# wangty537/raft_optical_flow

Hardware: AMD Instinct MI355X
Metric: image-pairs/s at Sintel 436x1024, 32 iters; corr-lookup GB/s vs HBM peak (higher is better)
Workload: dtype fp32 (convs: f16x3 split MFMA, fp32 accumulate); 1 GPU; RAFT-full inference, 436x1024 padded to 440x1024, 1 pair(s)/GPU/step, iters=32, all-pairs corr, hipGraph; global_batch=1, parallelism=frame-pair sharding x1

## Files before the change

### raft_optical_flow_amd/csrc/lookup_conv.hip

```cpp
#include "lookup_common.hpp"

namespace raft {
namespace {

constexpr int LC_TH = 2, LC_TW = 16, LC_M = 32;
constexpr int LC_R = 4, LC_L = 4, LC_RD = 9;
constexpr int LC_NTAP = LC_L * LC_RD * LC_RD;
constexpr int LC_KS = (LC_NTAP + 31) / 32;
constexpr int LC_N = 256;
constexpr int LC_F1N = 128;
constexpr int LC_F1K = 7, LC_F1KK = 49;
constexpr int LC_F1KS = (2 * LC_F1KK + 31) / 32;
constexpr int LC_FPH = LC_TH + LC_F1K - 1, LC_FPW = LC_TW + LC_F1K - 1;
constexpr int LC_PX = 4;

constexpr int LC_A_BYTES = LC_KS * LC_M * 128;
constexpr int LC_A1_BYTES = LC_F1KS * LC_M * 128;
constexpr int LC_FL_BYTES = LC_FPH * LC_FPW * 8;
constexpr int LC_PATCH_FLOATS = 16 * patch_rs<4>();
constexpr int LC_PATCH_BYTES = 8 * 2 * LC_PATCH_FLOATS * 4;
constexpr int LC_YT_BYTES = 8 * LC_PX * LC_L * LC_RD * 16;
constexpr int LC_OFF_A1 = LC_A_BYTES, LC_OFF_FL = LC_OFF_A1 + LC_A1_BYTES, LC_OFF_PATCH = LC_OFF_FL + LC_FL_BYTES,
              LC_OFF_YT = LC_OFF_PATCH + LC_PATCH_BYTES, LC_LDS = LC_OFF_YT + LC_YT_BYTES;
static_assert(LC_LDS <= 160 * 1024, "LDS budget");

struct LookupConvArgs {
  LookupArgs a;
  const h8* wfrag;
  const float* bias;
  float* out;
  int out_ld;
  int* out_flag;
  const h8* f1frag;
  const float* f1bias;
  float* f1out;
  int f1out_ld;
  int* f1flag;
  int tx_n, ty_n;
  int span_slot;
};

constexpr int LC_SPAN_SLOTS = 256;
__device__ unsigned long long g_lc_span[2 * LC_SPAN_SLOTS];
int g_lc_span_next = -1;

__device__ __forceinline__ void wave_sync() {
  __builtin_amdgcn_fence(__ATOMIC_RELEASE, "wavefront");
  __builtin_amdgcn_wave_barrier();
  __builtin_amdgcn_fence(__ATOMIC_ACQUIRE, "wavefront");
}

template <bool X3, bool BF>
__device__ __forceinline__ void split1(float x, _Float16& hi, _Float16& lo) {
  if constexpr (BF) {
    hi = __builtin_bit_cast(_Float16, (__bf16)x);
  } else {
    hi = (_Float16)x;
    if constexpr (X3) lo = (_Float16)(x - (float)hi);
  }
}

#ifdef LC_STAMPS
__device__ unsigned long long g_lcstamp[16 * 16384];
__device__ __forceinline__ unsigned long long lc_clock() {
  unsigned long long t;
  __builtin_amdgcn_sched_barrier(0);
  asm volatile("s_memtime %0\n\ts_waitcnt lgkmcnt(0)" : "=s"(t)::"memory");
  __builtin_amdgcn_sched_barrier(0);
  return t;
}
__device__ __forceinline__ unsigned long long lc_real() {
  unsigned long long t;
  __builtin_amdgcn_sched_barrier(0);
  asm volatile("s_memrealtime %0\n\ts_waitcnt lgkmcnt(0)" : "=s"(t)::"memory");
  __builtin_amdgcn_sched_barrier(0);
  return t;
}
#define LC_STAMP(k) lc_t[k] = lc_clock()
#else
#define LC_STAMP(k)
#endif

template <int PREC>
__global__ __launch_bounds__(512) void lookup_conv_kernel(LookupConvArgs g) {
#ifdef LC_STAMPS
  unsigned long long lc_t[10];
  const unsigned long long lc_r0 = lc_real();
  LC_STAMP(0);
#endif
  constexpr bool X3 = PREC == RAFT_PREC_F16X3;
  constexpr bool BF = PREC == RAFT_PREC_BF16;
  constexpr int NT = X3 ? 4 : 2;
  constexpr int R = LC_R, RD = LC_RD, WD = 2 * R + 2, RS = patch_rs<4>();
  __shared__ __attribute__((aligned(1024))) char smem[LC_LDS];
  const LookupArgs& a = g.a;
  const int lane = threadIdx.x & 63;
  const int wv = __builtin_amdgcn_readfirstlane(threadIdx.x >> 6);
  const int tile = xcd_tile(blockIdx.x, gridDim.x);
  if (g.span_slot >= 0 && threadIdx.x == 0)
    atomicMin(&g_lc_span[2 * g.span_slot], (unsigned long long)__builtin_amdgcn_s_memrealtime());
  const int per = g.tx_n * g.ty_n;
  const int b = tile / per, sr = tile - b * per;
  const int y0 = (sr / g.tx_n) * LC_TH, x0 = (sr % g.tx_n) * LC_TW;
  const int H = a.H, W = a.W, P = H * W;

  constexpr int LC_PF = 3;
  constexpr int PF = LC_PF;
  h8 wb[PF + 1][NT];
  auto load_w = [&](int j, h8 (&dst)[NT]) {
    const h8* wf = j < LC_KS ? g.wfrag + ((j * (LC_N / 32) + wv) * 4) * 64
                             : g.f1frag + (((j - LC_KS) * (LC_F1N / 32) + wv) * 4) * 64;
#pragma unroll
    for (int t = 0; t < NT; ++t) dst[t] = wf[t * 64 + lane];
  };

  const int ti = lane >> 4, tj = (lane >> 2) & 3, rr = lane & 3;
  const int lrow = ti * 4 + rr;
  int lth[LC_L], ltw[LC_L];
  unsigned lmsz[LC_L];
  const float* lbs[LC_L];
#pragma unroll
  for (int l = 0; l < LC_L; ++l) {
    lth[l] = a.lv[l].th;
    ltw[l] = a.lv[l].tw;
    lmsz[l] = (unsigned)a.lv[l].mapsz;
    lbs[l] = a.lbase[l];
  }
  float px_x[LC_PX], px_y[LC_PX];
  int px_gp[LC_PX];
  bool px_ok[LC_PX];
#pragma unroll
  for (int k = 0; k < LC_PX; ++k) {
    const int mk = LC_PX * wv + k;
    const int yy = y0 + (mk >> 4), xx = x0 + (mk & 15);
    const bool ok = yy < H && xx < W;
    px_ok[k] = ok;
    px_gp[k] = ok ? b * P + yy * W + xx : b * P;
  }
  {
    int gk = px_gp[0];
#pragma unroll
    for (int k = 1; k < LC_PX; ++k) gk = (lane & 3) == k ? px_gp[k] : gk;
    const float cx = a.coords[2L * gk], cy = a.coords[2L * gk + 1];
#pragma unroll
    for (int k = 0; k < LC_PX; ++k) {
      px_x[k] = __int_as_float(__builtin_amdgcn_readlane(__float_as_int(cx), k));
      px_y[k] = __int_as_float(__builtin_amdgcn_readlane(__float_as_int(cy), k));
    }
  }
#ifdef LC_STAMPS
  asm volatile("" ::"v"(px_x[0]), "v"(px_y[LC_PX - 1]));
  LC_STAMP(7);
#endif
  const bool col = lane < LC_L * RD;
  int lq = 0;
#pragma unroll
  for (int k = 1; k < LC_L; ++k) lq += lane >= k * RD ? 1 : 0;
  const int l = col ? lq : 0;
  const int ix = lane - l * RD;
  const f32x4 prm = a.prm[l];
  const int fi = threadIdx.x;
  const int fyy = y0 - 3 + fi / LC_FPW, fxx = x0 - 3 + fi % LC_FPW;
  const bool fin = fi < LC_FPH * LC_FPW && (unsigned)fyy < (unsigned)H && (unsigned)fxx < (unsigned)W;
  f32x2 fc = {0.f, 0.f};
  if (fin) fc = *reinterpret_cast<const f32x2*>(a.coords + 2L * ((long)b * P + fyy * W + fxx));
  const int m = lane & 31, h = lane >> 5;
  const float c1b = g.bias ? g.bias[32 * wv + m] : 0.f;
  const float f1b = (wv < 4 && g.f1bias) ? g.f1bias[32 * wv + m] : 0.f;
  asm volatile("" ::"v"(prm), "v"(c1b), "v"(f1b), "v"(fc));

  __builtin_amdgcn_sched_barrier(0);
  f32x4 v[LC_PX][LC_L];
  bool off32 = true;
  const unsigned nmaps = (unsigned)(a.B * P);
#pragma unroll
  for (int l = 0; l < LC_L; ++l) off32 &= (unsigned long long)nmaps * lmsz[l] * 4ull < 0x7FFFFFF0ull;
  if (off32) {
    __amdgpu_buffer_rsrc_t rsl[LC_L];
    unsigned lano[LC_L], lmsz4[LC_L];
#pragma unroll
    for (int l = 0; l < LC_L; ++l) {
      rsl[l] = __builtin_amdgcn_make_buffer_rsrc(const_cast<float*>(lbs[l]), (short)0, (int)(nmaps * lmsz[l] * 4u),
                                                 0x00020000);
      lano[l] = __umul24((unsigned)ti, (unsigned)(64 * ltw[l])) + 16u * (unsigned)(lane & 15);
      lmsz4[l] = lmsz[l] * 4u;
    }
    int t_sb, t_row, t_col;
    {
      const int ik = (lane >> 2) & 3, il = lane & 3;
      float fx = px_x[0], fy = px_y[0];
      int gpk = px_gp[0];
      bool okk = px_ok[0];
#pragma unroll
      for (int k = 1; k < LC_PX; ++k) {
        fx = ik == k ? px_x[k] : fx;
        fy = ik == k ? px_y[k] : fy;
        gpk = ik == k ? px_gp[k] : gpk;
        okk = ik == k ? px_ok[k] : okk;
      }
      int thl = lth[0], twl = ltw[0];
      unsigned msl = lmsz4[0];
#pragma unroll
      for (int l = 1; l < LC_L; ++l) {
        thl = il == l ? lth[l] : thl;
        twl = il == l ? ltw[l] : twl;
        msl = il == l ? lmsz4[l] : msl;
      }
      const int wx0 = (floor_origin(fx) >> il) - R, wy0 = (floor_origin(fy) >> il) - R;
      const int tyo = wy0 >> 2, txo = wx0 >> 2;
      const int ntx = ((wx0 + WD - 1) >> 2) - txo + 1;
      const int rlo = max(wy0, 0), rhi = min(wy0 + WD, 4 * thl);
      const int clo = max(txo, 0), chi = min(txo + ntx, twl);
      const int rn = okk ? max(rhi - rlo, 0) : 0, cn = max(chi - clo, 0);
      t_sb = (int)((unsigned)gpk * msl + (unsigned)(tyo * twl + txo) * 64u);
      t_row = ((rlo - 4 * tyo) & 0xFFFF) | (rn << 16);
      t_col = ((clo - txo) & 0xFFFF) | (cn << 16);
    }
#pragma unroll
    for (int k = 0; k < LC_PX; ++k) {
#pragma unroll
      for (int l = 0; l < LC_L; ++l) {
        const unsigned sb = (unsigned)__builtin_amdgcn_readlane(t_sb, 4 * k + l);
        const int rp = __builtin_amdgcn_readlane(t_row, 4 * k + l), cp = __builtin_amdgcn_readlane(t_col, 4 * k + l);
        const bool tok = ((unsigned)(lrow - (rp & 0xFFFF)) < (unsigned)(rp >> 16)) &
                         ((unsigned)(tj - (cp & 0xFFFF)) < (unsigned)(cp >> 16));
        unsigned offv = sb + lano[l];
        asm volatile("" : "+v"(offv));
        const unsigned off = tok ? offv : 0x80000000u;
        v[k][l] = __builtin_bit_cast(f32x4, __builtin_amdgcn_raw_buffer_load_b128(rsl[l], off, 0, 0));
      }
    }
  } else {
    int t_lo, t_hi, t_row, t_col;
    {
      const int ik = (lane >> 2) & 3, il = lane & 3;
      float fx = px_x[0], fy = px_y[0];
      int gpk = px_gp[0];
      bool okk = px_ok[0];
#pragma unroll
      for (int k = 1; k < LC_PX; ++k) {
        fx = ik == k ? px_x[k] : fx;
        fy = ik == k ? px_y[k] : fy;
        gpk = ik == k ? px_gp[k] : gpk;
        okk = ik == k ? px_ok[k] : okk;
      }
      int thl = lth[0], twl = ltw[0];
      unsigned msl = lmsz[0];
      const float* bsl = lbs[0];
#pragma unroll
      for (int l = 1; l < LC_L; ++l) {
        thl = il == l ? lth[l] : thl;
        twl = il == l ? ltw[l] : twl;
        msl = il == l ? lmsz[l] : msl;
        bsl = il == l ? lbs[l] : bsl;
      }
      const int wx0 = (floor_origin(fx) >> il) - R, wy0 = (floor_origin(fy) >> il) - R;
      const int tyo = wy0 >> 2, txo = wx0 >> 2;
      const int ntx = ((wx0 + WD - 1) >> 2) - txo + 1;
      const int rlo = max(wy0, 0), rhi = min(wy0 + WD, 4 * thl);
      const int clo = max(txo, 0), chi = min(txo + ntx, twl);
      const int rn = okk ? max(rhi - rlo, 0) : 0, cn = max(chi - clo, 0);
      const float* wbase = bsl + (long)((unsigned long long)(unsigned)gpk * msl) + ((long)tyo * twl + txo) * 16;
      const unsigned long long wa = reinterpret_cast<unsigned long long>(wbase);
      t_lo = (int)(unsigned)wa;
      t_hi = (int)(unsigned)(wa >> 32);
      t_row = ((rlo - 4 * tyo) & 0xFFFF) | (rn << 16);
      t_col = ((clo - txo) & 0xFFFF) | (cn << 16);
    }
#pragma unroll
    for (int k = 0; k < LC_PX; ++k) {
#pragma unroll
      for (int l = 0; l < LC_L; ++l) {
        const unsigned lo = (unsigned)__builtin_amdgcn_readlane(t_lo, 4 * k + l);
        const unsigned hi = (unsigned)__builtin_amdgcn_readlane(t_hi, 4 * k + l);
        const int rp = __builtin_amdgcn_readlane(t_row, 4 * k + l), cp = __builtin_amdgcn_readlane(t_col, 4 * k + l);
        const bool tok = ((unsigned)(lrow - (rp & 0xFFFF)) < (unsigned)(rp >> 16)) &
                         ((unsigned)(tj - (cp & 0xFFFF)) < (unsigned)(cp >> 16));
        const float* wbase = reinterpret_cast<const float*>(((unsigned long long)hi << 32) | lo);
        const __amdgpu_buffer_rsrc_t rs =
            __builtin_amdgcn_make_buffer_rsrc(const_cast<float*>(wbase), (short)0, 0x7FFFFFFF, 0x00020000);
        unsigned offv = __umul24((unsigned)ti, (unsigned)(64 * ltw[l])) + 16u * (unsigned)(lane & 15);
        asm volatile("" : "+v"(offv));
        const unsigned off = tok ? offv : 0x80000000u;
        v[k][l] = __builtin_bit_cast(f32x4, __builtin_amdgcn_raw_buffer_load_b128(rs, off, 0, 0));
      }
    }
  }
  LC_STAMP(1);
  int4* ytab = reinterpret_cast<int4*>(smem + LC_OFF_YT) + wv * LC_PX * LC_L * RD;
  int xw[LC_PX], xi[LC_PX];
  float xt[LC_PX];
  bool onp[LC_PX];
#pragma unroll
  for (int k = 0; k < LC_PX; ++k) {
    const float s = __builtin_ldexpf(1.0f, -l);
    const int xf = __builtin_amdgcn_readfirstlane(floor_origin(px_x[k]));
    const int yf = __builtin_amdgcn_readfirstlane(floor_origin(px_y[k]));
    axis_entry<R>(px_x[k] * s, xf >> l, ix, prm[0], prm[1], xw[k], xt[k], xi[k]);
    int yw, yi;
    float yt;
    axis_entry<R, true>(px_y[k] * s, yf >> l, ix, prm[2], prm[3], yw, yt, yi);
    onp[k] = xw[k] >= 0 && yw >= 0;
    if (col) ytab[k * LC_L * RD + lane] = int4{yw >= 0 ? yw * RS * 4 : yw, __float_as_int(yt), __float_as_int(1.0f - yt), yi};
  }
  float2* fl = reinterpret_cast<float2*>(smem + LC_OFF_FL);
  if (fi < LC_FPH * LC_FPW) {
    float2 fv = {0.f, 0.f};
    if (fin) {
      fv.x = fc[0] - (float)fxx;
      fv.y = fc[1] - (float)fyy;
    }
    fl[fi] = fv;
  }
  LC_STAMP(2);

#pragma unroll
  for (int j = 0; j < PF; ++j) load_w(j, wb[j]);
  char* Abase = smem;
  bool big = false;
  auto patch_of = [&](int k) {
    return reinterpret_cast<float*>(smem + LC_OFF_PATCH) + (wv * 2 + (k & 1)) * LC_PATCH_FLOATS;
  };
  const int cbase = l * RD * RD + ix * RD;
  auto taps = [&](int k, float (&val)[RD]) {
    const float* patch = patch_of(k);
    const int4* yt = ytab + k * LC_L * RD;
    const float ex = 1.0f - xt[k];
    const int xwk = xw[k];
    if (__all(!col || onp[k])) {
      if (col) {
        const char* p0 = reinterpret_cast<const char*>(&patch[pidx<4>(0, xwk, l)]);
        const char* p1 = reinterpret_cast<const char*>(&patch[pidx<4>(0, xwk + 1, l)]);
        auto at = [](const char* bp, int byte) { return *reinterpret_cast<const float*>(bp + byte); };
        int ro[RD];
        float tyv[RD];
        bool cons = true;
#pragma unroll
        for (int iy = 0; iy < RD; ++iy) {
          const int2 ye = *reinterpret_cast<const int2*>(&yt[l * RD + iy]);
          ro[iy] = ye.x;
          tyv[iy] = __int_as_float(ye.y);
        }
#pragma unroll
        for (int iy = 1; iy < RD; ++iy) cons &= ro[iy] == ro[0] + iy * (4 * RS);
        if (__all(cons)) {
          const char* q0 = p0 + ro[0];
          const char* q1 = p1 + ro[0];
          float a0[RD + 1], a1[RD + 1];
#pragma unroll
          for (int r = 0; r <= RD; ++r) {
            a0[r] = at(q0, r * (4 * RS));
            a1[r] = at(q1, r * (4 * RS));
          }
#pragma unroll
          for (int iy = 0; iy < RD; ++iy) {
            const float ty = tyv[iy], sS = 1.0f - ty;
            const f32x2 c0 = {a0[iy], a0[iy + 1]}, c1 = {a1[iy], a1[iy + 1]};
            const f32x2 hh = __builtin_elementwise_fma(c0, (f32x2){ex, ex}, c1 * (f32x2){xt[k], xt[k]});
            val[iy] = fmaf(sS, hh.x, ty * hh.y);
          }
        } else {
#pragma unroll
          for (int iy = 0; iy < RD; ++iy) {
            const float ty = tyv[iy], sS = 1.0f - ty;
            const f32x2 c0 = {at(p0, ro[iy]), at(p0, ro[iy] + 4 * RS)}, c1 = {at(p1, ro[iy]), at(p1, ro[iy] + 4 * RS)};
            const f32x2 hh = __builtin_elementwise_fma(c0, (f32x2){ex, ex}, c1 * (f32x2){xt[k], xt[k]});
            val[iy] = fmaf(sS, hh.x, ty * hh.y);
          }
        }
      }
    } else if (col) {
      unsigned deferred = 0;
#pragma unroll
      for (int iy = 0; iy < RD; ++iy) {
        const int4 ye = yt[l * RD + iy];
        const int yw2 = ye.x;
        const float ty = __int_as_float(ye.y), sS = __int_as_float(ye.z);
        const bool on = (xwk | yw2) >= 0;
        const bool nan = xwk == NAN_POS || yw2 == NAN_POS;
        const int r0 = on ? yw2 / (4 * RS) : 0, c0 = on ? xwk : 0;
        const float vv = patch[pidx<4>(r0, c0, l)] * (sS * ex) + patch[pidx<4>(r0, c0 + 1, l)] * (sS * xt[k]) +
                         patch[pidx<4>(r0 + 1, c0, l)] * (ty * ex) + patch[pidx<4>(r0 + 1, c0 + 1, l)] * (ty * xt[k]);
        val[iy] = nan ? __builtin_nanf("") : vv;
        deferred |= (!on && !nan) ? 1u << iy : 0u;
      }
      if (deferred != 0) {
        const Level& lvl = a.lv[l];
        const float* mp = a.pyr + lvl.off + (long)px_gp[k] * lvl.mapsz;
        auto at = [&](int yy, int xx) {
          return ((unsigned)yy < (unsigned)lvl.h && (unsigned)xx < (unsigned)lvl.w) ? mp[tiled_index(yy, xx, lvl.tw)]
                                                                                    : 0.f;
        };
#pragma unroll
        for (int iy = 0; iy < RD; ++iy) {
          if (!((deferred >> iy) & 1u)) continue;
          const int4 ye = yt[l * RD + iy];
          const int yi = ye.w;
          const float ty = __int_as_float(ye.y), sS = __int_as_float(ye.z);
          val[iy] = at(yi, xi[k]) * (sS * ex) + at(yi, xi[k] + 1) * (sS * xt[k]) + at(yi + 1, xi[k]) * (ty * ex) +
                    at(yi + 1, xi[k] + 1) * (ty * xt[k]);
        }
      }
    }
  };
  auto write_row = [&](int k, const float (&val)[RD]) {
    const int mk = LC_PX * wv + k;
    const int sw = (mk >> 1) & 7;
    if (col) {
      const int par = cbase & 1;
      float vv[RD];
#pragma unroll
      for (int iy = 0; iy < RD; ++iy) {
        vv[iy] = px_ok[k] ? val[iy] : 0.f;
        big |= fabsf(vv[iy]) > RAFT_RANGE_LIMIT;
      }
      auto at_c = [&](int c, int half) {
        const int j = c >> 5, kk = c & 31;
        return Abase + j * (LC_M * 128) + mk * 128 + (((4 * half + (kk >> 3)) ^ sw) << 4) + 2 * (kk & 7);
      };
#pragma unroll
      for (int q = 0; q < 4; ++q) {
        const float a0 = par ? vv[2 * q + 1] : vv[2 * q], a1 = par ? vv[2 * q + 2] : vv[2 * q + 1];
        _Float16 h0, l0, h1, l1;
        split1<X3, BF>(a0, h0, l0);
        split1<X3, BF>(a1, h1, l1);
        const int c = cbase + 2 * q + par;
        *reinterpret_cast<h2*>(at_c(c, 0)) = h2{h0, h1};
        if constexpr (X3) *reinterpret_cast<h2*>(at_c(c, 1)) = h2{l0, l1};
      }
      {
        const float a = par ? vv[0] : vv[RD - 1];
        _Float16 hs, ls;
        split1<X3, BF>(a, hs, ls);
        const int c = cbase + (par ? 0 : RD - 1);
        *reinterpret_cast<_Float16*>(at_c(c, 0)) = hs;
        if constexpr (X3) *reinterpret_cast<_Float16*>(at_c(c, 1)) = ls;
      }
    } else if (lane - LC_L * RD < 32 * LC_KS - LC_NTAP) {
      const int c = LC_NTAP + lane - LC_L * RD;
      const int j = c >> 5, kk = c & 31;
      char* rb = Abase + j * (LC_M * 128) + mk * 128;
      *reinterpret_cast<_Float16*>(rb + (((kk >> 3) ^ sw) << 4) + 2 * (kk & 7)) = (_Float16)0.f;
      if constexpr (X3) *reinterpret_cast<_Float16*>(rb + (((4 + (kk >> 3)) ^ sw) << 4) + 2 * (kk & 7)) = (_Float16)0.f;
    }
    if (a.flow && lane < 2 && px_ok[k]) {
      const int p = px_gp[k] - b * P;
      const float gcoord = lane == 0 ? (float)(p % W) : (float)(p / W);
      a.flow[(long)px_gp[k] * a.flow_ld + lane] = (lane == 0 ? px_x[k] : px_y[k]) - gcoord;
    }
  };
#pragma unroll
  for (int k = 0; k < LC_PX; k += 2) {
#pragma unroll
    for (int lv_ = 0; lv_ < LC_L; ++lv_) {
      *reinterpret_cast<f32x4*>(&patch_of(k)[pidx<4>(lrow, tj * 4, lv_)]) = v[k][lv_];
      *reinterpret_cast<f32x4*>(&patch_of(k + 1)[pidx<4>(lrow, tj * 4, lv_)]) = v[k + 1][lv_];
    }
    wave_sync();
    float va[RD], vb[RD];
    taps(k, va);
    taps(k + 1, vb);
    write_row(k, va);
    write_row(k + 1, vb);
    wave_sync();
  }
  if (a.range_flag && big) *a.range_flag = 1;
  LC_STAMP(3);
  __syncthreads();
  {
    const int mm = threadIdx.x >> 4, q = threadIdx.x & 15;
    const int py = mm >> 4, px = mm & 15;
    float e[8];
#pragma unroll
    for (int i = 0; i < 8; ++i) {
      const int k = 8 * q + i, t = k >> 1;
      const int dy = t / LC_F1K, dx = t - dy * LC_F1K;
      const float2 fv = fl[(py + (k < 2 * LC_F1KK ? dy : 0)) * LC_FPW + px + (k < 2 * LC_F1KK ? dx : 0)];
      e[i] = k < 2 * LC_F1KK ? ((k & 1) ? fv.y : fv.x) : 0.f;
    }
    h8 hi, lo;
    split8<X3, BF>(f32x4{e[0], e[1], e[2], e[3]}, f32x4{e[4], e[5], e[6], e[7]}, hi, lo);
    const int j = q >> 2, qd = q & 3, sw = (mm >> 1) & 7;
    char* row = smem + LC_OFF_A1 + j * (LC_M * 128) + mm * 128;
    *reinterpret_cast<h8*>(row + ((qd ^ sw) << 4)) = hi;
    if constexpr (X3) *reinterpret_cast<h8*>(row + (((4 + qd) ^ sw) << 4)) = lo;
  }
  __syncthreads();
  LC_STAMP(4);

  const int sw = (m >> 1) & 7;
  f32x16 acc = {}, accx = {}, facc = {}, faccx = {};
  const bool f1w = wv < LC_F1N / 32;
  struct AF {
    h8 ah[2], al[2];
  };
  auto read_af = [&](const char* A, AF& f) {
    const char* row = A + m * 128;
#pragma unroll
    for (int qq = 0; qq < 2; ++qq) {
      f.ah[qq] = *reinterpret_cast<const h8*>(row + (((2 * h + qq) ^ sw) << 4));
      if constexpr (X3) f.al[qq] = *reinterpret_cast<const h8*>(row + (((4 + 2 * h + qq) ^ sw) << 4));
    }
  };
  auto mfma_af = [&](const AF& f, const h8 (&B)[NT], f32x16& c, f32x16& cx) {
#pragma unroll
    for (int qq = 0; qq < 2; ++qq) {
      if constexpr (BF) {
        c = __builtin_amdgcn_mfma_f32_32x32x16_bf16(__builtin_bit_cast(bf8, f.ah[qq]), __builtin_bit_cast(bf8, B[qq]),
                                                    c, 0, 0, 0);
      } else {
        c = __builtin_amdgcn_mfma_f32_32x32x16_f16(f.ah[qq], B[qq], c, 0, 0, 0);
      }
      if constexpr (X3) {
        cx = __builtin_amdgcn_mfma_f32_32x32x16_f16(f.ah[qq], B[2 + qq], cx, 0, 0, 0);
        c = __builtin_amdgcn_mfma_f32_32x32x16_f16(f.al[qq], B[qq], c, 0, 0, 0);
      }
    }
  };
  auto load_w_any = [&](int j, h8 (&dst)[NT]) {
    const int wq = j < LC_KS ? wv : (wv < LC_F1N / 32 ? wv : LC_F1N / 32 - 1);
    const h8* wf = j < LC_KS ? g.wfrag + ((j * (LC_N / 32) + wq) * 4) * 64
                             : g.f1frag + (((j - LC_KS) * (LC_F1N / 32) + wq) * 4) * 64;
#pragma unroll
    for (int t = 0; t < NT; ++t) dst[t] = wf[t * 64 + lane];
  };
  constexpr int NRA = X3 ? 4 : 2, NMA = X3 ? 6 : 2;
  auto groups = [&](bool loads) {
    if (loads) __builtin_amdgcn_sched_group_barrier(0x020, NT, 0);
#pragma unroll
    for (int i = 0; i < NMA; ++i) {
      if (i < NRA) __builtin_amdgcn_sched_group_barrier(0x100, 1, 0);
      __builtin_amdgcn_sched_group_barrier(0x008, 1, 0);
    }
  };
  AF af[2];
  read_af(Abase, af[0]);
#pragma unroll
  for (int j = 0; j < LC_KS; ++j) {
    __builtin_amdgcn_sched_barrier(0);
    if (j + PF < LC_KS + LC_F1KS) load_w_any(j + PF, wb[(j + PF) % (PF + 1)]);
    read_af(j + 1 < LC_KS ? Abase + (j + 1) * (LC_M * 128) : smem + LC_OFF_A1, af[(j + 1) & 1]);
    mfma_af(af[j & 1], wb[j % (PF + 1)], acc, accx);
    groups(j + PF < LC_KS + LC_F1KS);
    __builtin_amdgcn_sched_barrier(0);
  }
  if (f1w) {
#pragma unroll
    for (int j = LC_KS; j < LC_KS + LC_F1KS; ++j) {
      __builtin_amdgcn_sched_barrier(0);
      if (j + PF < LC_KS + LC_F1KS) load_w_any(j + PF, wb[(j + PF) % (PF + 1)]);
      if (j + 1 < LC_KS + LC_F1KS) read_af(smem + LC_OFF_A1 + (j + 1 - LC_KS) * (LC_M * 128), af[(j + 1) & 1]);
      mfma_af(af[j & 1], wb[j % (PF + 1)], facc, faccx);
      __builtin_amdgcn_sched_barrier(0);
    }
  }
  if constexpr (X3) {
#pragma unroll
    for (int r = 0; r < 16; ++r) {
      acc[r] += accx[r] * (1.0f / SPLIT_SCALE);
      facc[r] += faccx[r] * (1.0f / SPLIT_SCALE);
    }
  }
#ifdef LC_STAMPS
  asm volatile("" ::"v"(acc[0]), "v"(acc[15]), "v"(facc[0]));
#endif
  LC_STAMP(5);

  auto store = [&](const f32x16& c, float bias, float* out, int ld, int n, int* flag) {
    bool obig = false;
#pragma unroll
    for (int r = 0; r < 16; ++r) {
      const int mm = (r & 3) + 8 * (r >> 2) + 4 * h;
      const int yy = y0 + (mm >> 4), xx = x0 + (mm & 15);
      const float o = fmaxf(c[r] + bias, 0.f);
      if (yy < H && xx < W) {
        obig |= o > RAFT_RANGE_LIMIT;
        out[((long)b * P + yy * W + xx) * ld + n] = o;
      }
    }
    if (flag && obig) *flag = 1;
  };
  store(acc, c1b, g.out, g.out_ld, 32 * wv + m, g.out_flag);
  if (wv < LC_F1N / 32) store(facc, f1b, g.f1out, g.f1out_ld, 32 * wv + m, g.f1flag);
  if (g.span_slot >= 0) {
    __builtin_amdgcn_s_waitcnt(0);
    __syncthreads();
    if (threadIdx.x == 0)
      atomicMax(&g_lc_span[2 * g.span_slot + 1], (unsigned long long)__builtin_amdgcn_s_memrealtime());
  }
#ifdef LC_STAMPS
  __builtin_amdgcn_s_waitcnt(0);
  LC_STAMP(6);
  const unsigned long long lc_r1 = lc_real();
  const unsigned wid = blockIdx.x * 8 + wv;
  if (lane == 0 && wid < 16384) {
    unsigned long long* gs = g_lcstamp + wid * 16;
    gs[0] = lc_r0;
    gs[1] = lc_r1;
    for (int k = 0; k < 7; ++k) gs[2 + k] = lc_t[k];
    gs[9] = lc_t[7];
  }
#endif
}

__global__ void lookup_conv_pack_kernel(const h8* __restrict__ split, int k_steps, int nsub, h8* __restrict__ out) {
  const int i = blockIdx.x * blockDim.x + threadIdx.x;
  const int total = k_steps * nsub * 4 * 64;
  if (i >= total) return;
  const int lane = i & 63, t = (i >> 6) & 3, rest = i >> 8;
  const int s = rest % nsub, j = rest / nsub;
  const int n = 32 * s + (lane & 31), hh = lane >> 5, qq = t & 1, lo = t >> 1;
  out[i] = split[((long)n * k_steps + j) * 8 + lo * 4 + 2 * hh + qq];
}

}
}

using namespace raft;

#ifdef LC_STAMPS
extern "C" int raft_debug_lcstamps(unsigned long long* host, int n) {
  return (int)hipMemcpyFromSymbol(host, HIP_SYMBOL(g_lcstamp), sizeof(unsigned long long) * (size_t)n);
}
#endif

extern "C" size_t raft_lookup_conv_weight_floats(int n, int k_pad) {
  if (n <= 0 || n % 32 || k_pad <= 0) return 0;
  return (size_t)((k_pad + 31) / 32) * (size_t)n * 32;
}

extern "C" int raft_lookup_conv_pack_weight(const void* split_weight, int n_pad, int k_pad, int n, void* out,
                                            raft_stream_t stream) {
  RAFT_REQUIRE(split_weight && out && n > 0 && n % 32 == 0 && n <= n_pad && k_pad > 0 && k_pad % 32 == 0,
               "raft_lookup_conv_pack_weight: bad arguments");
  RAFT_REQUIRE((((uintptr_t)split_weight | (uintptr_t)out) & 15) == 0, "raft_lookup_conv_pack_weight: 16-B alignment");
  const int ks = k_pad / 32, nsub = n / 32;
  const int total = ks * nsub * 256;
  hipLaunchKernelGGL(lookup_conv_pack_kernel, dim3((unsigned)cdiv(total, 256)), dim3(256), 0, as_stream(stream),
                     reinterpret_cast<const h8*>(split_weight), ks, nsub, reinterpret_cast<h8*>(out));
  return check_launch("raft_lookup_conv_pack_weight");
}

extern "C" int raft_corr_lookup_conv(const float* pyramid, int B, int H, int W, int L, int radius, const float* coords,
                                     float* flow_out, int flow_ld, int* range_flag, int precision,
                                     const void* c1_weight, const float* c1_bias, int c1_n, float* c1_out,
                                     int c1_out_ld, int* c1_range_flag, const void* f1_weight, const float* f1_bias,
                                     int f1_n, int f1_k, float* f1_out, int f1_out_ld, int* f1_range_flag,
                                     raft_stream_t stream) {
  RAFT_REQUIRE(L == LC_L && radius == LC_R, "raft_corr_lookup_conv: radius 4 and 4 levels only (got %d, %d)", radius,
               L);
  RAFT_REQUIRE(c1_n == LC_N && f1_n == LC_F1N && f1_k == LC_F1K,
               "raft_corr_lookup_conv: convc1 256 / convf1 128 outputs, convf1 7x7 only");
  RAFT_REQUIRE(precision == RAFT_PREC_F16X3 || precision == RAFT_PREC_F16 || precision == RAFT_PREC_BF16,
               "raft_corr_lookup_conv: precision must be F16X3, F16 or BF16 (got %d)", precision);
  RAFT_REQUIRE(c1_weight && c1_out && c1_out_ld >= c1_n && f1_weight && f1_out && f1_out_ld >= f1_n,
               "raft_corr_lookup_conv: bad conv arguments");
  RAFT_REQUIRE((((uintptr_t)c1_weight | (uintptr_t)f1_weight) & 15) == 0 && ((uintptr_t)coords & 7) == 0,
               "raft_corr_lookup_conv: 16-B aligned weights, 8-B aligned coords");
  LookupConvArgs g;
  int rc = lookup_args(g.a, pyramid, B, H, W, L, radius, coords, 0, c1_out, LC_NTAP, 0, flow_out, flow_ld, range_flag);
  if (rc) return rc;
  g.wfrag = reinterpret_cast<const h8*>(c1_weight);
  g.bias = c1_bias;
  g.out = c1_out;
  g.out_ld = c1_out_ld;
  g.out_flag = c1_range_flag;
  g.f1frag = reinterpret_cast<const h8*>(f1_weight);
  g.f1bias = f1_bias;
  g.f1out = f1_out;
  g.f1out_ld = f1_out_ld;
  g.f1flag = f1_range_flag;
  g.tx_n = cdiv(W, LC_TW);
  g.ty_n = cdiv(H, LC_TH);
  hipStreamCaptureStatus cap = hipStreamCaptureStatusNone;
  const bool capturing = hipStreamIsCapturing(as_stream(stream), &cap) == hipSuccess && cap != hipStreamCaptureStatusNone;
  g.span_slot = !capturing && g_lc_span_next >= 0 && g_lc_span_next < LC_SPAN_SLOTS ? g_lc_span_next++ : -1;
  const long nt = (long)B * g.tx_n * g.ty_n;
  RAFT_REQUIRE(nt < (1L << 31), "raft_corr_lookup_conv: grid too large");
  hipStream_t s = as_stream(stream);
  const dim3 grid((unsigned)nt);
  if (precision == RAFT_PREC_F16X3)
    hipLaunchKernelGGL(lookup_conv_kernel<RAFT_PREC_F16X3>, grid, dim3(512), 0, s, g);
  else if (precision == RAFT_PREC_F16)
    hipLaunchKernelGGL(lookup_conv_kernel<RAFT_PREC_F16>, grid, dim3(512), 0, s, g);
  else
    hipLaunchKernelGGL(lookup_conv_kernel<RAFT_PREC_BF16>, grid, dim3(512), 0, s, g);
  return check_launch("raft_corr_lookup_conv");
}

extern "C" int raft_debug_launch_span(int enable) {
  using namespace raft;
  unsigned long long init[2 * LC_SPAN_SLOTS];
  for (int i = 0; i < LC_SPAN_SLOTS; ++i) {
    init[2 * i] = ~0ull;
    init[2 * i + 1] = 0ull;
  }
  const hipError_t e = hipMemcpyToSymbol(HIP_SYMBOL(g_lc_span), init, sizeof(init));
  if (e != hipSuccess) return set_error((int)e, "raft_debug_launch_span: %s", hipGetErrorString(e));
  g_lc_span_next = enable ? 0 : -1;
  return 0;
}
extern "C" int raft_debug_launch_span_read(unsigned long long* host, int n) {
  using namespace raft;
  RAFT_REQUIRE(host && n > 0 && n <= 2 * LC_SPAN_SLOTS, "raft_debug_launch_span_read: bad arguments");
  const hipError_t e = hipMemcpyFromSymbol(host, HIP_SYMBOL(g_lc_span), sizeof(unsigned long long) * (size_t)n);
  if (e != hipSuccess) return set_error((int)e, "raft_debug_launch_span_read: %s", hipGetErrorString(e));
  return 0;
}
```

Baseline: 139.9 image-pairs/s.

## Split lookup-conv tile across 16 waves using 16x16 MFMA tiles

Raises the fused corr-lookup + conv kernel from 8 to 16 waves per block. Each wave now handles 2 pixels instead of 4 and a 16-channel output slice instead of 32. The convolution switches from 32x32x16 to 16x16x32 MFMA with a new weight-fragment lane mapping, and output stores become 4-wide vectors. The f1 A-tile pack now uses half-width writes. The goal is more latency hiding and parallelism per tile, at the cost of more waves competing for LDS, duplicated weight loads across wave pairs, and a per-wave single patch buffer with extra sched barriers.

After: 142.0 image-pairs/s (median of 6 runs). 1.01x the previous value.

```diff
diff --git a/raft_optical_flow_amd/csrc/lookup_conv.hip b/raft_optical_flow_amd/csrc/lookup_conv.hip
--- a/raft_optical_flow_amd/csrc/lookup_conv.hip
+++ b/raft_optical_flow_amd/csrc/lookup_conv.hip
@@ -7,19 +7,21 @@
 constexpr int LC_R = 4, LC_L = 4, LC_RD = 9;
 constexpr int LC_NTAP = LC_L * LC_RD * LC_RD;
 constexpr int LC_KS = (LC_NTAP + 31) / 32;
+constexpr int LC_WV = 16;
 constexpr int LC_N = 256;
 constexpr int LC_F1N = 128;
 constexpr int LC_F1K = 7, LC_F1KK = 49;
 constexpr int LC_F1KS = (2 * LC_F1KK + 31) / 32;
 constexpr int LC_FPH = LC_TH + LC_F1K - 1, LC_FPW = LC_TW + LC_F1K - 1;
-constexpr int LC_PX = 4;
+constexpr int LC_PX = LC_M / LC_WV;
+static_assert(LC_PX == 2 && LC_N == 16 * LC_WV && LC_F1N == 8 * LC_WV, "wave roles");
 
 constexpr int LC_A_BYTES = LC_KS * LC_M * 128;
 constexpr int LC_A1_BYTES = LC_F1KS * LC_M * 128;
 constexpr int LC_FL_BYTES = LC_FPH * LC_FPW * 8;
 constexpr int LC_PATCH_FLOATS = 16 * patch_rs<4>();
-constexpr int LC_PATCH_BYTES = 8 * 2 * LC_PATCH_FLOATS * 4;
-constexpr int LC_YT_BYTES = 8 * LC_PX * LC_L * LC_RD * 16;
+constexpr int LC_PATCH_BYTES = LC_WV * LC_PATCH_FLOATS * 4;
+constexpr int LC_YT_BYTES = LC_WV * LC_PX * LC_L * LC_RD * 16;
 constexpr int LC_OFF_A1 = LC_A_BYTES, LC_OFF_FL = LC_OFF_A1 + LC_A1_BYTES, LC_OFF_PATCH = LC_OFF_FL + LC_FL_BYTES,
               LC_OFF_YT = LC_OFF_PATCH + LC_PATCH_BYTES, LC_LDS = LC_OFF_YT + LC_YT_BYTES;
 static_assert(LC_LDS <= 160 * 1024, "LDS budget");
@@ -82,7 +84,7 @@
 #endif
 
 template <int PREC>
-__global__ __launch_bounds__(512) void lookup_conv_kernel(LookupConvArgs g) {
+__global__ __launch_bounds__(64 * LC_WV) void lookup_conv_kernel(LookupConvArgs g) {
 #ifdef LC_STAMPS
   unsigned long long lc_t[10];
   const unsigned long long lc_r0 = lc_real();
@@ -90,7 +92,7 @@
 #endif
   constexpr bool X3 = PREC == RAFT_PREC_F16X3;
   constexpr bool BF = PREC == RAFT_PREC_BF16;
-  constexpr int NT = X3 ? 4 : 2;
+  constexpr int NT = X3 ? 2 : 1;
   constexpr int R = LC_R, RD = LC_RD, WD = 2 * R + 2, RS = patch_rs<4>();
   __shared__ __attribute__((aligned(1024))) char smem[LC_LDS];
   const LookupArgs& a = g.a;
@@ -107,11 +109,14 @@
   constexpr int LC_PF = 3;
   constexpr int PF = LC_PF;
   h8 wb[PF + 1][NT];
+  const int n16 = lane & 15, q4 = lane >> 4;
+  const int wlane = (q4 & 1) * 64 + 32 * (q4 >> 1) + 16 * (wv & 1) + n16;
   auto load_w = [&](int j, h8 (&dst)[NT]) {
-    const h8* wf = j < LC_KS ? g.wfrag + ((j * (LC_N / 32) + wv) * 4) * 64
-                             : g.f1frag + (((j - LC_KS) * (LC_F1N / 32) + wv) * 4) * 64;
-#pragma unroll
-    for (int t = 0; t < NT; ++t) dst[t] = wf[t * 64 + lane];
+    const int f1s = wv < LC_F1N / 16 ? wv >> 1 : LC_F1N / 32 - 1;
+    const h8* wf = j < LC_KS ? g.wfrag + ((j * (LC_N / 32) + (wv >> 1)) * 4) * 64
+                             : g.f1frag + (((j - LC_KS) * (LC_F1N / 32) + f1s) * 4) * 64;
+#pragma unroll
+    for (int t = 0; t < NT; ++t) dst[t] = wf[t * 128 + wlane];
   };
 
   const int ti = lane >> 4, tj = (lane >> 2) & 3, rr = lane & 3;
@@ -140,7 +145,7 @@
   {
     int gk = px_gp[0];
 #pragma unroll
-    for (int k = 1; k < LC_PX; ++k) gk = (lane & 3) == k ? px_gp[k] : gk;
+    for (int k = 1; k < LC_PX; ++k) gk = (lane & (LC_PX - 1)) == k ? px_gp[k] : gk;
     const float cx = a.coords[2L * gk], cy = a.coords[2L * gk + 1];
 #pragma unroll
     for (int k = 0; k < LC_PX; ++k) {
@@ -164,10 +169,7 @@
   const bool fin = fi < LC_FPH * LC_FPW && (unsigned)fyy < (unsigned)H && (unsigned)fxx < (unsigned)W;
   f32x2 fc = {0.f, 0.f};
   if (fin) fc = *reinterpret_cast<const f32x2*>(a.coords + 2L * ((long)b * P + fyy * W + fxx));
-  const int m = lane & 31, h = lane >> 5;
-  const float c1b = g.bias ? g.bias[32 * wv + m] : 0.f;
-  const float f1b = (wv < 4 && g.f1bias) ? g.f1bias[32 * wv + m] : 0.f;
-  asm volatile("" ::"v"(prm), "v"(c1b), "v"(f1b), "v"(fc));
+  asm volatile("" ::"v"(prm), "v"(fc));
 
   __builtin_amdgcn_sched_barrier(0);
   f32x4 v[LC_PX][LC_L];
@@ -187,7 +189,7 @@
     }
     int t_sb, t_row, t_col;
     {
-      const int ik = (lane >> 2) & 3, il = lane & 3;
+      const int ik = (lane >> 2) & (LC_PX - 1), il = lane & 3;
       float fx = px_x[0], fy = px_y[0];
       int gpk = px_gp[0];
       bool okk = px_ok[0];
@@ -233,7 +235,7 @@
   } else {
     int t_lo, t_hi, t_row, t_col;
     {
-      const int ik = (lane >> 2) & 3, il = lane & 3;
+      const int ik = (lane >> 2) & (LC_PX - 1), il = lane & 3;
       float fx = px_x[0], fy = px_y[0];
       int gpk = px_gp[0];
       bool okk = px_ok[0];
@@ -314,16 +316,12 @@
   }
   LC_STAMP(2);
 
-#pragma unroll
-  for (int j = 0; j < PF; ++j) load_w(j, wb[j]);
   char* Abase = smem;
   bool big = false;
-  auto patch_of = [&](int k) {
-    return reinterpret_cast<float*>(smem + LC_OFF_PATCH) + (wv * 2 + (k & 1)) * LC_PATCH_FLOATS;
-  };
+  float* const wpatch = reinterpret_cast<float*>(smem + LC_OFF_PATCH) + wv * LC_PATCH_FLOATS;
   const int cbase = l * RD * RD + ix * RD;
   auto taps = [&](int k, float (&val)[RD]) {
-    const float* patch = patch_of(k);
+    const float* patch = wpatch;
     const int4* yt = ytab + k * LC_L * RD;
     const float ex = 1.0f - xt[k];
     const int xwk = xw[k];
@@ -383,6 +381,7 @@
                          patch[pidx<4>(r0 + 1, c0, l)] * (ty * ex) + patch[pidx<4>(r0 + 1, c0 + 1, l)] * (ty * xt[k]);
         val[iy] = nan ? __builtin_nanf("") : vv;
         deferred |= (!on && !nan) ? 1u << iy : 0u;
+        __builtin_amdgcn_sched_barrier(0);
       }
       if (deferred != 0) {
         const Level& lvl = a.lv[l];
@@ -450,79 +449,78 @@
     }
   };
 #pragma unroll
-  for (int k = 0; k < LC_PX; k += 2) {
-#pragma unroll
-    for (int lv_ = 0; lv_ < LC_L; ++lv_) {
-      *reinterpret_cast<f32x4*>(&patch_of(k)[pidx<4>(lrow, tj * 4, lv_)]) = v[k][lv_];
-      *reinterpret_cast<f32x4*>(&patch_of(k + 1)[pidx<4>(lrow, tj * 4, lv_)]) = v[k + 1][lv_];
-    }
+  for (int k = 0; k < LC_PX; ++k) {
+    if (k == LC_PX - 1) {
+#pragma unroll
+      for (int j = 0; j < PF; ++j) load_w(j, wb[j]);
+    }
+#pragma unroll
+    for (int lv_ = 0; lv_ < LC_L; ++lv_) *reinterpret_cast<f32x4*>(&wpatch[pidx<4>(lrow, tj * 4, lv_)]) = v[k][lv_];
     wave_sync();
-    float va[RD], vb[RD];
+    float va[RD];
     taps(k, va);
-    taps(k + 1, vb);
     write_row(k, va);
-    write_row(k + 1, vb);
     wave_sync();
   }
   if (a.range_flag && big) *a.range_flag = 1;
+  float c1b[4], f1b[4];
+#pragma unroll
+  for (int i = 0; i < 4; ++i) {
+    c1b[i] = g.bias ? g.bias[16 * wv + 4 * q4 + i] : 0.f;
+    f1b[i] = (wv < LC_F1N / 16 && g.f1bias) ? g.f1bias[16 * wv + 4 * q4 + i] : 0.f;
+  }
   LC_STAMP(3);
   __syncthreads();
   {
-    const int mm = threadIdx.x >> 4, q = threadIdx.x & 15;
+    const int mm = threadIdx.x >> 5, q = threadIdx.x & 31;
     const int py = mm >> 4, px = mm & 15;
-    float e[8];
-#pragma unroll
-    for (int i = 0; i < 8; ++i) {
-      const int k = 8 * q + i, t = k >> 1;
+    float e[4];
+#pragma unroll
+    for (int i = 0; i < 4; ++i) {
+      const int k = 4 * q + i, t = k >> 1;
       const int dy = t / LC_F1K, dx = t - dy * LC_F1K;
       const float2 fv = fl[(py + (k < 2 * LC_F1KK ? dy : 0)) * LC_FPW + px + (k < 2 * LC_F1KK ? dx : 0)];
       e[i] = k < 2 * LC_F1KK ? ((k & 1) ? fv.y : fv.x) : 0.f;
     }
     h8 hi, lo;
-    split8<X3, BF>(f32x4{e[0], e[1], e[2], e[3]}, f32x4{e[4], e[5], e[6], e[7]}, hi, lo);
-    const int j = q >> 2, qd = q & 3, sw = (mm >> 1) & 7;
-    char* row = smem + LC_OFF_A1 + j * (LC_M * 128) + mm * 128;
-    *reinterpret_cast<h8*>(row + ((qd ^ sw) << 4)) = hi;
-    if constexpr (X3) *reinterpret_cast<h8*>(row + (((4 + qd) ^ sw) << 4)) = lo;
+    split8<X3, BF>(f32x4{e[0], e[1], e[2], e[3]}, f32x4{0.f, 0.f, 0.f, 0.f}, hi, lo);
+    const int j = q >> 3, qd = (q >> 1) & 3, sw = (mm >> 1) & 7;
+    char* row = smem + LC_OFF_A1 + j * (LC_M * 128) + mm * 128 + 8 * (q & 1);
+    *reinterpret_cast<h4*>(row + ((qd ^ sw) << 4)) = h4{hi[0], hi[1], hi[2], hi[3]};
+    if constexpr (X3) *reinterpret_cast<h4*>(row + (((4 + qd) ^ sw) << 4)) = h4{lo[0], lo[1], lo[2], lo[3]};
   }
   __syncthreads();
   LC_STAMP(4);
 
-  const int sw = (m >> 1) & 7;
-  f32x16 acc = {}, accx = {}, facc = {}, faccx = {};
-  const bool f1w = wv < LC_F1N / 32;
+  f32x4 acc[2] = {}, accx[2] = {}, facc[2] = {}, faccx[2] = {};
+  const bool f1w = wv < LC_F1N / 16;
   struct AF {
     h8 ah[2], al[2];
   };
+  const int arow = n16 * 128, asw = (n16 >> 1) & 7;
   auto read_af = [&](const char* A, AF& f) {
-    const char* row = A + m * 128;
-#pragma unroll
-    for (int qq = 0; qq < 2; ++qq) {
-      f.ah[qq] = *reinterpret_cast<const h8*>(row + (((2 * h + qq) ^ sw) << 4));
-      if constexpr (X3) f.al[qq] = *reinterpret_cast<const h8*>(row + (((4 + 2 * h + qq) ^ sw) << 4));
-    }
-  };
-  auto mfma_af = [&](const AF& f, const h8 (&B)[NT], f32x16& c, f32x16& cx) {
-#pragma unroll
-    for (int qq = 0; qq < 2; ++qq) {
-      if constexpr (BF) {
-        c = __builtin_amdgcn_mfma_f32_32x32x16_bf16(__builtin_bit_cast(bf8, f.ah[qq]), __builtin_bit_cast(bf8, B[qq]),
-                                                    c, 0, 0, 0);
-      } else {
-        c = __builtin_amdgcn_mfma_f32_32x32x16_f16(f.ah[qq], B[qq], c, 0, 0, 0);
-      }
-      if constexpr (X3) {
-        cx = __builtin_amdgcn_mfma_f32_32x32x16_f16(f.ah[qq], B[2 + qq], cx, 0, 0, 0);
-        c = __builtin_amdgcn_mfma_f32_32x32x16_f16(f.al[qq], B[qq], c, 0, 0, 0);
-      }
-    }
-  };
-  auto load_w_any = [&](int j, h8 (&dst)[NT]) {
-    const int wq = j < LC_KS ? wv : (wv < LC_F1N / 32 ? wv : LC_F1N / 32 - 1);
-    const h8* wf = j < LC_KS ? g.wfrag + ((j * (LC_N / 32) + wq) * 4) * 64
-                             : g.f1frag + (((j - LC_KS) * (LC_F1N / 32) + wq) * 4) * 64;
-#pragma unroll
-    for (int t = 0; t < NT; ++t) dst[t] = wf[t * 64 + lane];
+#pragma unroll
+    for (int r = 0; r < 2; ++r) {
+      const char* row = A + r * (16 * 128) + arow;
+      f.ah[r] = *reinterpret_cast<const h8*>(row + ((q4 ^ asw) << 4));
+      if constexpr (X3) f.al[r] = *reinterpret_cast<const h8*>(row + (((4 + q4) ^ asw) << 4));
+    }
+  };
+  auto mfma1 = [&](const h8& w, const h8& x, f32x4& c) {
+    if constexpr (BF)
+      c = __builtin_amdgcn_mfma_f32_16x16x32_bf16(__builtin_bit_cast(bf8, w), __builtin_bit_cast(bf8, x), c, 0, 0, 0);
+    else
+      c = __builtin_amdgcn_mfma_f32_16x16x32_f16(w, x, c, 0, 0, 0);
+  };
+  auto mfma_af = [&](const AF& f, const h8 (&B)[NT], f32x4 (&c)[2], f32x4 (&cx)[2]) {
+    mfma1(B[0], f.ah[0], c[0]);
+    mfma1(B[0], f.ah[1], c[1]);
+    if constexpr (X3) {
+      mfma1(B[NT - 1], f.ah[0], cx[0]);
+      mfma1(B[NT - 1], f.ah[1], cx[1]);
+      mfma1(B[0], f.al[0], c[0]);
+      mfma1(B[0], f.al[1], c[1]);
+    }
   };
   constexpr int NRA = X3 ? 4 : 2, NMA = X3 ? 6 : 2;
   auto groups = [&](bool loads) {
@@ -538,7 +536,7 @@
 #pragma unroll
   for (int j = 0; j < LC_KS; ++j) {
     __builtin_amdgcn_sched_barrier(0);
-    if (j + PF < LC_KS + LC_F1KS) load_w_any(j + PF, wb[(j + PF) % (PF + 1)]);
+    if (j + PF < LC_KS + LC_F1KS) load_w(j + PF, wb[(j + PF) % (PF + 1)]);
     read_af(j + 1 < LC_KS ? Abase + (j + 1) * (LC_M * 128) : smem + LC_OFF_A1, af[(j + 1) & 1]);
     mfma_af(af[j & 1], wb[j % (PF + 1)], acc, accx);
     groups(j + PF < LC_KS + LC_F1KS);
@@ -548,7 +546,7 @@
 #pragma unroll
     for (int j = LC_KS; j < LC_KS + LC_F1KS; ++j) {
       __builtin_amdgcn_sched_barrier(0);
-      if (j + PF < LC_KS + LC_F1KS) load_w_any(j + PF, wb[(j + PF) % (PF + 1)]);
+      if (j + PF < LC_KS + LC_F1KS) load_w(j + PF, wb[(j + PF) % (PF + 1)]);
       if (j + 1 < LC_KS + LC_F1KS) read_af(smem + LC_OFF_A1 + (j + 1 - LC_KS) * (LC_M * 128), af[(j + 1) & 1]);
       mfma_af(af[j & 1], wb[j % (PF + 1)], facc, faccx);
       __builtin_amdgcn_sched_barrier(0);
@@ -556,32 +554,41 @@
   }
   if constexpr (X3) {
 #pragma unroll
-    for (int r = 0; r < 16; ++r) {
+    for (int r = 0; r < 2; ++r) {
       acc[r] += accx[r] * (1.0f / SPLIT_SCALE);
       facc[r] += faccx[r] * (1.0f / SPLIT_SCALE);
     }
   }
 #ifdef LC_STAMPS
-  asm volatile("" ::"v"(acc[0]), "v"(acc[15]), "v"(facc[0]));
+  asm volatile("" ::"v"(acc[0]), "v"(acc[1]), "v"(facc[0]));
 #endif
   LC_STAMP(5);
 
-  auto store = [&](const f32x16& c, float bias, float* out, int ld, int n, int* flag) {
+  auto store = [&](const f32x4 (&c)[2], const float (&bias)[4], float* out, int ld, int n, int* flag) {
     bool obig = false;
-#pragma unroll
-    for (int r = 0; r < 16; ++r) {
-      const int mm = (r & 3) + 8 * (r >> 2) + 4 * h;
-      const int yy = y0 + (mm >> 4), xx = x0 + (mm & 15);
-      const float o = fmaxf(c[r] + bias, 0.f);
+    const bool vec = ((ld & 3) | (int)(reinterpret_cast<uintptr_t>(out) & 15)) == 0;
+#pragma unroll
+    for (int r = 0; r < 2; ++r) {
+      const int yy = y0 + r, xx = x0 + n16;
+      f32x4 o;
+#pragma unroll
+      for (int i = 0; i < 4; ++i) o[i] = fmaxf(c[r][i] + bias[i], 0.f);
       if (yy < H && xx < W) {
-        obig |= o > RAFT_RANGE_LIMIT;
-        out[((long)b * P + yy * W + xx) * ld + n] = o;
+#pragma unroll
+        for (int i = 0; i < 4; ++i) obig |= o[i] > RAFT_RANGE_LIMIT;
+        float* dst = out + ((long)b * P + yy * W + xx) * ld + n;
+        if (vec) {
+          *reinterpret_cast<f32x4*>(dst) = o;
+        } else {
+#pragma unroll
+          for (int i = 0; i < 4; ++i) dst[i] = o[i];
+        }
       }
     }
     if (flag && obig) *flag = 1;
   };
-  store(acc, c1b, g.out, g.out_ld, 32 * wv + m, g.out_flag);
-  if (wv < LC_F1N / 32) store(facc, f1b, g.f1out, g.f1out_ld, 32 * wv + m, g.f1flag);
+  store(acc, c1b, g.out, g.out_ld, 16 * wv + 4 * q4, g.out_flag);
+  if (f1w) store(facc, f1b, g.f1out, g.f1out_ld, 16 * wv + 4 * q4, g.f1flag);
   if (g.span_slot >= 0) {
     __builtin_amdgcn_s_waitcnt(0);
     __syncthreads();
@@ -592,7 +599,7 @@
   __builtin_amdgcn_s_waitcnt(0);
   LC_STAMP(6);
   const unsigned long long lc_r1 = lc_real();
-  const unsigned wid = blockIdx.x * 8 + wv;
+  const unsigned wid = blockIdx.x * LC_WV + wv;
   if (lane == 0 && wid < 16384) {
     unsigned long long* gs = g_lcstamp + wid * 16;
     gs[0] = lc_r0;
@@ -680,11 +687,11 @@
   hipStream_t s = as_stream(stream);
   const dim3 grid((unsigned)nt);
   if (precision == RAFT_PREC_F16X3)
-    hipLaunchKernelGGL(lookup_conv_kernel<RAFT_PREC_F16X3>, grid, dim3(512), 0, s, g);
+    hipLaunchKernelGGL(lookup_conv_kernel<RAFT_PREC_F16X3>, grid, dim3(64 * LC_WV), 0, s, g);
   else if (precision == RAFT_PREC_F16)
-    hipLaunchKernelGGL(lookup_conv_kernel<RAFT_PREC_F16>, grid, dim3(512), 0, s, g);
+    hipLaunchKernelGGL(lookup_conv_kernel<RAFT_PREC_F16>, grid, dim3(64 * LC_WV), 0, s, g);
   else
-    hipLaunchKernelGGL(lookup_conv_kernel<RAFT_PREC_BF16>, grid, dim3(512), 0, s, g);
+    hipLaunchKernelGGL(lookup_conv_kernel<RAFT_PREC_BF16>, grid, dim3(64 * LC_WV), 0, s, g);
   return check_launch("raft_corr_lookup_conv");
 }
 
```
